# onucharles/tensorized-rnn

Measured on AMD Instinct MI355X. Metric: timesteps/sec/GPU (batch=64) TT-LSTM h=256 ncores=3 rank=8, higher is better.
Workload: dtype f32 (2xfp16 operands, fp32 accumulate)

## Files before the change

### tensorized-rnn_amd/csrc/ttrnn_f10_dev.h

```cpp
#pragma once
#include <hip/hip_runtime.h>
#include "ttrnn_core.h"
#include "ttrnn_mfma.h"
#include "ttrnn_split.h"
#include "ttrnn_f10.h"

namespace ttrnn {

template <class S, int KS>
constexpr size_t f10_lds_bytes() {
  return 2 * sizeof(float) * F10<S>::H + 2 * 3 * 2 * (size_t)F10<S>::H + 2 * 3 * (size_t)F10<S>::PLANE +
         (KS == 2 ? F10<S>::MT * 64 * sizeof(f32x4) : 0);
}

template <class S>
__device__ __forceinline__ void f10_load_w2(xbf8& a1, xbf8& a2, const float* packed, int mt, int lane) {
  using F = F10<S>;
  const int r = lane & 15, q = lane >> 4;
  const float* W2 = packed + woff_of<S>(2);
#pragma unroll
  for (int e = 0; e < 8; ++e) {
    __bf16 p0, p1, p2;
    split3(e < F::J2 ? W2[e * F::M2 + 16 * mt + r] : 0.f, p0, p1, p2);
    a1[e] = (q & 1) ? p1 : p0;
// ... 221 lines not shown
#pragma unroll
  for (int e = 0; e < 4; ++e) d[e] = ln.live ? d[e] : 0u;
  const xh8 bfrag = __builtin_bit_cast(xh8, u32x4{d[0], d[1], d[2], d[3]});
  f32x4 acc[NP];
#pragma unroll
  for (int p = 0; p < NP; ++p) acc[p] = __builtin_amdgcn_mfma_f32_16x16x32_f16(a1[p], bfrag, f32x4{0.f, 0.f, 0.f, 0.f}, 0, 0, 0);
#pragma unroll
  for (int p = 0; p < NP; ++p) acc[p] = __builtin_amdgcn_mfma_f32_16x16x32_f16(a2[p], bfrag, acc[p], 0, 0, 0);
#pragma unroll
  for (int p = 0; p < NP; ++p) store_split4_h(img, F::PLANE, ln.soff[p], acc[p]);
}
template <class S>
__device__ __forceinline__ void f10p_s2_lds(const xh8* afr, int lane, const F10pLane<S>& ln, unsigned pk, _Float16* img) {
  using F = F10<S>;
  constexpr int NP = F10P<S>::NP;
  unsigned d[4];
#pragma unroll
  for (int e = 0; e < 4; ++e) d[e] = (unsigned)__builtin_amdgcn_ds_bpermute(ln.gsrc + 4 * e, (int)pk);
#pragma unroll
  for (int e = 0; e < 4; ++e) d[e] = ln.live ? d[e] : 0u;
  const xh8 bfrag = __builtin_bit_cast(xh8, u32x4{d[0], d[1], d[2], d[3]});
  constexpr int GP = NP < 3 ? NP : 3;
  static_assert(NP % GP == 0, "pair groups");
#pragma unroll
  for (int p0 = 0; p0 < NP; p0 += GP) {
    xh8 fa[GP], fb[GP];
#pragma unroll
    for (int p = 0; p < GP; ++p) {
      fa[p] = afr[(2 * (p0 + p)) * 64 + lane];
      fb[p] = afr[(2 * (p0 + p) + 1) * 64 + lane];
    }
    f32x4 acc[GP];
#pragma unroll
    for (int p = 0; p < GP; ++p) acc[p] = __builtin_amdgcn_mfma_f32_16x16x32_f16(fa[p], bfrag, f32x4{0.f, 0.f, 0.f, 0.f}, 0, 0, 0);
#pragma unroll
    for (int p = 0; p < GP; ++p) acc[p] = __builtin_amdgcn_mfma_f32_16x16x32_f16(fb[p], bfrag, acc[p], 0, 0, 0);
#pragma unroll
    for (int p = 0; p < GP; ++p) store_split4_h(img, F::PLANE, ln.soff[p0 + p], acc[p]);
  }
}
__device__ __forceinline__ unsigned f10p_pack(float hscaled) {
  _Float16 p0, p1;
  split2h(hscaled, p0, p1);
  return (unsigned)__builtin_bit_cast(unsigned short, p0) | ((unsigned)__builtin_bit_cast(unsigned short, p1) << 16);
}

template <class S>
__global__ void __launch_bounds__(256) k_f10h_scale(const float* __restrict__ packed, int* __restrict__ hdr) {
  using F = F10<S>;
  static_assert(F::I2 <= 16 && F::R2 <= 16 && F::K % 64 == 0, "one workgroup (blockIdx.x) per row of the fused core: launch F::M of them");
  __shared__ unsigned mx[32];
  __shared__ int eu[16], ev[16];
  const int tid = threadIdx.x, lane = tid & 63, wave = tid >> 6;
  const float* W2 = packed + woff_of<S>(2);
  if (tid < 32) mx[tid] = 0u;
  __syncthreads();
  for (int i = tid; i < F::J2 * F::M2; i += 256)
    atomicMax(&mx[(i % F::M2) / F::R2], __float_as_uint(fabsf(W2[i])));
  __syncthreads();
  if (tid < 16) eu[tid] = tid < F::I2 ? -f10h_expo(__uint_as_float(mx[tid])) : 0;
  __syncthreads();
  for (int i = tid; i < F::J2 * F::M2; i += 256) {
    const int m2 = i % F::M2;
    atomicMax(&mx[16 + m2 % F::R2], __float_as_uint(fabsf(W2[i]) * ldexpf(1.f, eu[m2 / F::R2])));
  }
  __syncthreads();
  if (tid < 16) ev[tid] = tid < F::R2 ? -f10h_expo(__uint_as_float(mx[16 + tid])) : 0;
  __syncthreads();
  __shared__ float red[4];
  const int m = blockIdx.x;
  const int i0 = m / F::I1, i1 = m % F::I1;
  const float* W0 = packed + woff_of<S>(0);
  const float* W1 = packed + woff_of<S>(1);
  float best = 0.f;
  for (int k = tid; k < F::K; k += 256) {
    const int r2 = k % F::R2, row2 = k / F::R2;
    const int j1 = row2 % F::J1, j0 = row2 / F::J1;
    const float* w1p = W1 + (j1 * F::R2 + r2) * (F::I1 * F::R1) + i1 * F::R1;
    float v = 0.f;
    for (int r1 = 0; r1 < F::R1; ++r1) v = fmaf(W0[(j0 * F::R1 + r1) * F::I0 + i0], w1p[r1], v);
    best = fmaxf(best, fabsf(v) * ldexpf(1.f, -ev[r2]));
  }
#pragma unroll
  for (int o = 32; o > 0; o >>= 1) best = fmaxf(best, __shfl_xor(best, o));
  if (lane == 0) red[wave] = best;
  __syncthreads();
  if (tid == 0) hdr[F10H_EP + m] = 12 - f10h_expo(fmaxf(fmaxf(red[0], red[1]), fmaxf(red[2], red[3])));
  if (blockIdx.x == 0 && tid < 16) {
    hdr[F10H_EU + tid] = eu[tid];
    hdr[F10H_EV + tid] = ev[tid];
  }
}

static constexpr int F10T_ROW_EXP = 10;
static constexpr int F10T_ACC_EXP = 16;
static constexpr float F10T_HSC = 16.0f;
template <class S>
__device__ __forceinline__ int f10t_build_w10(xh8 (&w10)[8][2], const float* packed, const float* __restrict__ hdr, int wave, int lane) {
  using F = F10<S>;
  static_assert(F::R2 == 8 && F::J0 == 4 && F::J1 == 8 && F::R1 == 8 && F::M == 64 && F::MPG == 16, "H = 256, r = 8");
  const int c = lane & 15, q = lane >> 4;
  const int* ev = reinterpret_cast<const int*>(hdr) + F10H_EV;
  const int g = c & 3, m = F::MPG * g + 4 * wave + (c >> 2);
  const int i0 = m / F::I1, i1 = m % F::I1;
  const float* W0 = packed + woff_of<S>(0);
  const float* W1 = packed + woff_of<S>(1);
  float w0[F::R1];
#pragma unroll
  for (int r1 = 0; r1 < F::R1; ++r1) w0[r1] = W0[(q * F::R1 + r1) * F::I0 + i0];
  auto entry = [&](int e, int r2) {
    const float* w1p = W1 + (e * F::R2 + r2) * (F::I1 * F::R1) + i1 * F::R1;
    float v = 0.f;
#pragma unroll
    for (int r1 = 0; r1 < F::R1; ++r1) v = fmaf(w0[r1], w1p[r1], v);
    return v;
  };
  float best = 0.f;
#pragma unroll
  for (int r2 = 0; r2 < F::R2; ++r2) {
    float l1 = 0.f;
#pragma unroll
    for (int e = 0; e < 8; ++e) l1 += fabsf(entry(e, r2));
    l1 += __shfl_xor(l1, 16);
    l1 += __shfl_xor(l1, 32);
    best = fmaxf(best, l1 * ldexpf(1.f, -ev[r2]));
  }
  const int ept = F10T_ROW_EXP - f10h_expo(best);
  const float gf = g == 2 ? 2.8853900817779268f : -1.4426950408889634f;
#pragma unroll
  for (int r2 = 0; r2 < F::R2; ++r2) {
    const float sc = gf * ldexpf(1.f, ept - ev[r2]);
#pragma unroll
    for (int e = 0; e < 8; ++e) {
      _Float16 p0, p1;
      split2h_scaled(entry(e, r2), sc, p0, p1);
      w10[r2][0][e] = p0; w10[r2][1][e] = p1;
    }
  }
  return ept;
}
__device__ __forceinline__ F10hScales f10t_scales(const float* __restrict__ hdr, int ept_mine, int lane) {
  const int* e = reinterpret_cast<const int*>(hdr);
  const int c = lane & 15, q = lane >> 4;
  const int eu = e[F10H_EU + c];
  F10hScales r;
#pragma unroll
  for (int j = 0; j < 4; ++j) {
    const int s = __shfl(ept_mine, 4 * q + j) + eu + F10T_ACC_EXP;
    r.pre[j] = ldexpf(1.f, s);
    r.un[j] = ldexpf(1.f, -s);
  }
  return r;
}
template <class S>
__device__ __forceinline__ void f10t_load_g2(xh8 (&g2)[2][2], const float* packed, int lane, const float* __restrict__ hdr) {
  using F = F10<S>;
  const int c = lane & 15, q = lane >> 4;
  const float* W2 = packed + woff_of<S>(2);
  const int* e = reinterpret_cast<const int*>(hdr);
#pragma unroll
  for (int kb = 0; kb < 2; ++kb)
#pragma unroll
    for (int j = 0; j < 8; ++j) {
      const int r2 = 2 * kb + (j >> 2) + 4 * (q >> 1), j2 = 4 * (q & 1) + (j & 3);
      _Float16 p0, p1;
      split2h(W2[j2 * F::M2 + c * F::R2 + r2] * ldexpf(1.f, 12 + e[F10H_EU + c] + e[F10H_EV + r2]), p0, p1);
      g2[kb][0][j] = p0; g2[kb][1][j] = p1;
    }
}

}
```

### tensorized-rnn_amd/csrc/ttrnn_fast_f10t.hip

```cpp
#include <hip/hip_runtime.h>
#include <stdlib.h>
#include "ttrnn_core.h"
#include "ttrnn_launch.h"
#include "ttrnn_opts.h"
#include "ttrnn_mfma.h"
#include "ttrnn_split.h"
#include "ttrnn_f10.h"
#include "ttrnn_f10_dev.h"

namespace ttrnn {

static constexpr size_t F10T_LDS_BYTES = 2 * 2 * 8 * 32 * sizeof(_Float16) + 64;

template <class S, bool H0, bool OUT, bool IN1, bool DIAG = false>
__global__ void __launch_bounds__(256, 2) k_lstm_fwd_f10t(int B, int T, GinSrc gs, const float* __restrict__ h0,
                                                          const float* __restrict__ c0, const float* __restrict__ packed_hid,
                                                          const float* __restrict__ hdr,
                                                          const float* __restrict__ bias_hid, float* __restrict__ out,
                                                          float* __restrict__ hT, float* __restrict__ cT,
                                                          float* __restrict__ reserve) {
  static_assert(f10_ok<S>(), "shape not supported by the fused-core kernel");
  using F = F10<S>;
  static_assert(F::MT == 4 && F::ROWS2 == 32 && F::J2 == 8 && F::R2 == 8 && F::I2 == 16 && F::M == 64, "H = 256, r = 8");
  constexpr int H = F::H;
  constexpr int PAR = 2 * 8 * 32;

  extern __shared__ __attribute__((aligned(16))) unsigned char smem_t[];
  _Float16* himg = reinterpret_cast<_Float16*>(smem_t);
  float* scratch = reinterpret_cast<float*>(himg + 2 * PAR);

  const int tid = threadIdx.x, lane = tid & 63;
  const int wave = __builtin_amdgcn_readfirstlane(tid >> 6);
  xh8 w10[F::R2][2];
  const F10hScales fsc = f10t_scales(hdr, f10t_build_w10<S>(w10, packed_hid, hdr, wave, lane), lane);
  const float hsc = F10T_HSC;
  const f32x4 psc = fsc.pre, usc = fsc.un;
  const int c = lane & 15, q = lane >> 4;
  const size_t b = blockIdx.x;

  xh8 g2[2][2];
  f10t_load_g2<S>(g2, packed_hid, lane, hdr);

  const float* __restrict__ gin = gs.gin;
  const float* __restrict__ xs = reinterpret_cast<const float*>(gs.x);
  constexpr bool in1 = IN1;
  const int hd = (4 * wave + q) * F::I2 + c;
  const int hoff = (hd & 7) * 32 + (hd >> 3);
  float hst = H0 ? h0[b * H + hd] : 0.f;
  float cst = c0 ? c0[b * H + hd] : 0.f;
  float h0sc = 1.0f, h0un = 1.0f;
  if constexpr (H0) {
    const int e0 = f10h_h0_expo<4>(hst, scratch, wave, lane);
    h0sc = ldexpf(1.f, -e0); h0un = ldexpf(1.f, e0);
  }
  f32x4 bh = f32x4{0.f, 0.f, 0.f, 0.f}, gi = bh, vv = bh, bb = bh;
  const f32x4 gsc = f32x4{-1.4426950408889634f, 2.8853900817779268f, -1.4426950408889634f, -1.4426950408889634f} *
                    f32x4{psc[0], psc[2], psc[1], psc[3]};
  XChunk<float> xq;
  xq.cur = 0.f; xq.nxt = 0.f;
  if (in1) xq.init(xs, b * T, T, lane);
  if (bias_hid) bh = f32x4{bias_hid[hd], bias_hid[2 * H + hd], bias_hid[H + hd], bias_hid[3 * H + hd]};
  if (T > 0) {
    if (in1) {
      bb = *reinterpret_cast<const f32x4*>(gin + (H + hd) * 4);
      vv = (*reinterpret_cast<const f32x4*>(gin + hd * 4) - bb) * gsc;
      bb = (bb + bh) * gsc;
    } else {
      gi = *reinterpret_cast<const f32x4*>(gin + ((b * T) * H + hd) * 4);
    }
  }
  {
    _Float16 p0, p1;
    split2h(hst * (hsc * h0sc), p0, p1);
    himg[hoff] = p0; himg[256 + hoff] = p1;
  }
  __builtin_amdgcn_s_waitcnt(0x0F70);
  lds_barrier();

  unsigned long long seg[8] = {0, 0, 0, 0, 0, 0, 0, 0};
  unsigned long long last_ = 0;
  if constexpr (DIAG) last_ = stamp();
  f32x4 us_t = usc * h0un;
  float ps_t = h0sc;
  for (int t = 0; t < T; ++t) {
    const _Float16* hp = himg + (t & 1) * PAR;
    _Float16* hn = himg + ((t + 1) & 1) * PAR;
    const xh8 ha = *reinterpret_cast<const xh8*>(hp + c * 32 + 8 * q);
    f32x4 d[F::R2];
#pragma unroll
    for (int r = 0; r < F::R2; ++r) d[r] = __builtin_amdgcn_mfma_f32_16x16x32_f16(ha, w10[r][0], f32x4{0.f, 0.f, 0.f, 0.f}, 0, 0, 0);
#pragma unroll
    for (int r = 0; r < F::R2; ++r) d[r] = __builtin_amdgcn_mfma_f32_16x16x32_f16(ha, w10[r][1], d[r], 0, 0, 0);
    if constexpr (DIAG) {
#pragma unroll
      for (int r = 0; r < F::R2; ++r) asm volatile("" : "+v"(d[r]));
    }
    TT_STAMP(0)
    unsigned a0[2][4], a1[2][4];
#pragma unroll
    for (int p = 0; p < 4; ++p) {
      f32x4 s;
#pragma unroll
      for (int j = 0; j < 4; ++j) {
        const auto r = __builtin_amdgcn_permlane32_swap(__float_as_uint(d[p][j]), __float_as_uint(d[p + 4][j]), false, false);
        s[j] = __uint_as_float(r[0]) + __uint_as_float(r[1]);
      }
      split_pair_h(s[0], s[1], a0[p >> 1][2 * (p & 1)], a1[p >> 1][2 * (p & 1)]);
      split_pair_h(s[2], s[3], a0[p >> 1][2 * (p & 1) + 1], a1[p >> 1][2 * (p & 1) + 1]);
    }
    if constexpr (DIAG) {
#pragma unroll
      for (int kb = 0; kb < 2; ++kb)
#pragma unroll
        for (int j = 0; j < 4; ++j) asm volatile("" : "+v"(a0[kb][j]), "+v"(a1[kb][j]));
    }
    TT_STAMP(1)
    const size_t bt = b * T + t;
    f32x4 acc;
    {
      f32x4 pre = in1 ? bb + xq.at(t) * vv : (gi + bh) * gsc;
      if constexpr (H0) pre = pre * ps_t;
      f32x4 acc_lo = f32x4{0.f, 0.f, 0.f, 0.f}, acc_hi = f32x4{pre[0], pre[2], pre[1], pre[3]};
#pragma unroll
      for (int kb = 0; kb < 2; ++kb) {
        const xh8 d0 = __builtin_bit_cast(xh8, u32x4{a0[kb][0], a0[kb][1], a0[kb][2], a0[kb][3]});
        const xh8 d1 = __builtin_bit_cast(xh8, u32x4{a1[kb][0], a1[kb][1], a1[kb][2], a1[kb][3]});
        acc_lo = __builtin_amdgcn_mfma_f32_16x16x32_f16(d0, g2[kb][1], acc_lo, 0, 0, 0);
        acc_lo = __builtin_amdgcn_mfma_f32_16x16x32_f16(d1, g2[kb][0], acc_lo, 0, 0, 0);
        acc_hi = __builtin_amdgcn_mfma_f32_16x16x32_f16(d0, g2[kb][0], acc_hi, 0, 0, 0);
      }
      const f32x4 un = H0 ? us_t : usc;
      acc = acc_hi * un + acc_lo * un;
      if constexpr (DIAG) asm volatile("" : "+v"(acc));
    }
    TT_STAMP(2)
    const float ig = __builtin_amdgcn_rcpf(1.0f + __builtin_amdgcn_exp2f(acc[0]));
    const float fg = __builtin_amdgcn_rcpf(1.0f + __builtin_amdgcn_exp2f(acc[1]));
    const float gg = 1.0f - 2.0f * __builtin_amdgcn_rcpf(1.0f + __builtin_amdgcn_exp2f(acc[2]));
    const float og = __builtin_amdgcn_rcpf(1.0f + __builtin_amdgcn_exp2f(acc[3]));
    const float cy = fg * cst + ig * gg;
    const float hy = og * ftanh(cy);
    cst = cy;
    hst = hy;
    {
      _Float16 p0, p1;
      split2h(hy * hsc, p0, p1);
      hn[hoff] = p0; hn[256 + hoff] = p1;
    }
    if constexpr (OUT) out[bt * H + hd] = hy;
    if (reserve) {
      *reinterpret_cast<f32x4*>(reserve + res_gate(bt, H, hd)) = f32x4{ig, gg, fg, og};
      reserve[res_cell((size_t)B * T, bt, H, hd)] = cy;
    }
    if (!in1 && t + 1 < T) gi = *reinterpret_cast<const f32x4*>(gin + ((bt + 1) * H + hd) * 4);
    if (in1) xq.advance(xs, b * T, T, t, lane);
    us_t = usc; ps_t = 1.0f;
    TT_STAMP(3)
    lds_barrier();
    TT_STAMP(4)
  }
  if (hT) hT[b * H + hd] = hst;
  if (cT) cT[b * H + hd] = cst;
  if constexpr (DIAG) {
    if (lane == 0 && reserve && b < 8) {
      unsigned long long* dst = reinterpret_cast<unsigned long long*>(reserve) + (b * 8 + wave) * 8;
#pragma unroll
      for (int i = 0; i < 8; ++i) dst[i] = seg[i];
    }
  }
}

bool f10t_available(const RnnShape& rs) {
  if (opt(OPT_DEV2) & 2048) return false;
  return shape_matches<ShpH256R8L>(rs.hid_s) && rs.B <= device_cu_count();
}

int launch_rnn_fwd_f10_t(const RnnShape& rs, GinSrc gin, const void* h0, const void* c0, const float* packed_hid,
                         const void* ws, const float* bias_hid, void* out, void* hT, void* cT, float* reserve,
                         hipStream_t stream) {
  using S = ShpH256R8L;
  if (!shape_matches<S>(rs.hid_s)) return TTRNN_ERR_UNSUPPORTED;
  const float* hdr = reinterpret_cast<const float*>(ws);
  auto kern = gin.in1 ? (out ? (h0 ? k_lstm_fwd_f10t<S, true, true, true> : k_lstm_fwd_f10t<S, false, true, true>)
                             : (h0 ? k_lstm_fwd_f10t<S, true, false, true> : k_lstm_fwd_f10t<S, false, false, true>))
                      : (out ? (h0 ? k_lstm_fwd_f10t<S, true, true, false> : k_lstm_fwd_f10t<S, false, true, false>)
                             : (h0 ? k_lstm_fwd_f10t<S, true, false, false> : k_lstm_fwd_f10t<S, false, false, false>));
  if (opt(OPT_DIAG) && reserve && out && !h0)
    kern = gin.in1 ? k_lstm_fwd_f10t<S, false, true, true, true> : k_lstm_fwd_f10t<S, false, true, false, true>;
  hipLaunchKernelGGL(kern, dim3(rs.B), dim3(256), F10T_LDS_BYTES, stream, rs.B, rs.T, gin, (const float*)h0,
                     (const float*)c0, packed_hid, hdr, bias_hid, (float*)out, (float*)hT, (float*)cT, reserve);
  return hipGetLastError() == hipSuccess ? TTRNN_OK : TTRNN_ERR_LAUNCH;
}

}
```

### tensorized-rnn_amd/csrc/ttrnn_launch.h

```cpp
#pragma once
#include <hip/hip_runtime.h>
#include "ttrnn_core.h"

namespace ttrnn {

unsigned* device_status_ptr();


inline int device_cu_count() {
  static int cached[16] = {0};
  int dev = 0;
  if (hipGetDevice(&dev) != hipSuccess) {
    (void)hipGetLastError();
    return 256;
  }
  if (dev < 0 || dev >= 16) dev = 0;
  if (cached[dev] == 0) {
    int v = 256;
    if (hipDeviceGetAttribute(&v, hipDeviceAttributeMultiprocessorCount, dev) != hipSuccess) (void)hipGetLastError();
    cached[dev] = v > 0 ? v : 256;
  }
  return cached[dev];
}

int ensure_dynamic_lds(const void* fn, size_t bytes);
bool resident_at_once(const void* fn, int block_threads, size_t dyn_lds, long blocks);

struct GinSrc {
  const float* gin;
  const void* x;
  int in1;
  const int* run_if = nullptr;
  unsigned* status = nullptr;
};

struct LinPlan {
  int nb;
  int bs;
  int ss;
  int grid;
  bool w_lds;
  bool buf_global;
  bool buf_mixed;
  bool acc_lds;
  bool acc_slab;
  bool acc_fixed;
  size_t slab_off;
  size_t lds_bytes, ws_bytes;
};

struct RnnPlan {
  int nb, grid;
  bool w_lds, buf_global;
  size_t lds_bytes, ws_bytes;
};

LinPlan plan_ttlinear_fwd(const TtShape& s, int64_t n_rows);
LinPlan plan_ttlinear_bwd(const TtShape& s, int64_t n_rows, bool fixed_order = false);
RnnPlan plan_rnn_generic(const RnnShape& rs, bool backward);

const void* unit_rows_ptr(int dtype);
size_t in1_reduce_part_bytes(int out);
int launch_in1_reduce(int dtype, int dy_dtype, int64_t n_rows, int out, const void* x, const void* dy, float* dv,
                      float* db, float* part, hipStream_t stream);
int launch_pack(const TtShape& s, const void* const* cores, const int64_t* strides, int dtype, float* packed,
                hipStream_t stream);
int launch_pack2(const TtShape& sa, const void* const* cores_a, const int64_t* strides_a, float* packed_a,
                 const TtShape& sb, const void* const* cores_b, const int64_t* strides_b, float* packed_b, int dtype,
                 hipStream_t stream);
int launch_unpack(const TtShape& s, const float* packed_grad, void* const* grads, const int64_t* strides, int dtype,
                  hipStream_t stream);
int launch_ttlinear_fwd(const TtShape& s, const LinPlan& p, int dtype, int64_t n_rows, const float* packed,
                        const void* bias, const void* x, void* y, void* ws, hipStream_t stream, int ilv_h = 0,
                        int ilv_mode = 0, int epi = 0, float* aux = nullptr);
int launch_ttlinear_bwd(const TtShape& s, const LinPlan& p, int dtype, int dy_dtype, int64_t n_rows, const float* packed,
                        const void* x, const void* dy, void* dx, float* d_packed, float* d_bias, void* ws,
                        hipStream_t stream);
int launch_rnn_fwd_generic(const RnnShape& rs, const RnnPlan& p, int dtype, const void* x, const void* h0,
                           const void* c0, const float* packed_in, const void* bias_in, const float* packed_hid,
                           const void* bias_hid, void* out, void* hT, void* cT, float* reserve, void* ws,
                           hipStream_t stream, const int* lens = nullptr);
int launch_rnn_bwd_generic(const RnnShape& rs, const RnnPlan& p, int dtype, const void* out, const void* h0,
                           const void* c0, const float* packed_hid, const float* reserve, const void* d_out,
                           const void* d_hT, const void* d_cT, float* dg_in, float* dg_hid, void* d_h0, void* d_c0,
                           void* ws, hipStream_t stream, float* dstate = nullptr);

bool fast_rnn_fwd_available(const RnnShape& rs, int dtype);
int launch_rnn_fwd_fast(const RnnShape& rs, int dtype, GinSrc gin, const void* h0, const void* c0,
                        const float* packed_hid, const void* bias_hid, void* out, void* hT, void* cT, float* reserve,
                        hipStream_t stream);

bool fast_ttlinear_fwd_available(const TtShape& s, int dtype, int ilv_h);
int launch_ttlinear_fwd_fast(const TtShape& s, int dtype, bool y_f32, int64_t n_rows, const float* packed,
                             const void* bias, const void* x, void* y, int ilv_h, int ilv_mode, hipStream_t stream);

bool fast_rnn_fwd_bf16_available(const RnnShape& rs, int dtype);
int launch_rnn_fwd_bf16(const RnnShape& rs, GinSrc gin, const void* h0, const void* c0,
                        const float* packed_hid, const void* bias_hid, void* out, void* hT, void* cT, float* reserve,
                        hipStream_t stream);

bool f10_rnn_fwd_available(const RnnShape& rs, int dtype);
size_t f10_workspace_bytes(const RnnShape& rs, int dtype);
int launch_rnn_fwd_f10(const RnnShape& rs, GinSrc gin, const void* h0, const void* c0, const float* packed_hid,
                       const void* bias_hid, void* out, void* hT, void* cT, float* reserve, void* ws,
                       hipStream_t stream, int phase = 0);

bool f2_rnn_fwd_available(const RnnShape& rs, int dtype);
size_t f2_workspace_bytes(const RnnShape& rs, int dtype);
int launch_rnn_fwd_f2(const RnnShape& rs, GinSrc gin, const void* h0, const void* c0, const float* packed_hid,
                      const void* bias_hid, void* out, void* hT, void* cT, float* reserve, void* ws, hipStream_t stream, int phase);
bool f2_rnn_bwd_available(const RnnShape& rs, int dtype);
size_t f2_rnn_bwd_workspace_bytes(const RnnShape& rs, int dtype);
int launch_rnn_bwd_f2(const RnnShape& rs, const void* c0, const float* packed_hid, const float* reserve, const void* d_out,
                      const void* d_hT, const void* d_cT, float* dg_in, float* dg_hid, void* d_h0, void* d_c0, void* ws,
                      hipStream_t stream);

size_t f10gq_workspace_bytes();
bool f10gq_available(const RnnShape& rs, int dtype);
int launch_gru_fwd_f10gq(const RnnShape& rs, GinSrc gin, const void* h0, const float* packed_hid, const void* bias_hid,
                         void* out, void* hT, float* reserve, void* ws, hipStream_t stream, int phase);
bool f10_setup_available(const RnnShape& rs, int dtype);
int launch_f10_setup(const RnnShape& rs, const void* const* cores_in, const int64_t* strides_in, const void* bias_in,
                     const void* const* cores_hid, const int64_t* strides_hid, float* packed_in, float* packed_hid, float* gin,
                     void* ws, hipStream_t stream);
bool f10s_available(const RnnShape& rs, bool with_h0);
int launch_rnn_fwd_f10_s(const RnnShape& rs, GinSrc gin, const void* h0, const void* c0, const float* packed_hid, const void* ws,
                         const float* bias_hid, void* out, void* hT, void* cT, float* reserve, hipStream_t stream);
size_t f10gh_workspace_bytes(const RnnShape& rs);
bool f10gh_available(const RnnShape& rs, int dtype);
int launch_gru_fwd_f10gh(const RnnShape& rs, GinSrc gin, const void* h0, const float* packed_hid, const void* bias_hid, void* out,
                         void* hT, float* reserve, void* ws, hipStream_t stream, int phase);
bool f10n_available(const RnnShape& rs, int dtype);
size_t f10n_workspace_bytes(const RnnShape& rs);
int launch_lstm_fwd_f10n(const RnnShape& rs, GinSrc gin, const float* bilv, const void* h0, const void* c0, const float* packed_hid,
                         void* out, void* hT, void* cT, float* reserve, void* ws, hipStream_t stream);
bool f10g5_available(const RnnShape& rs, int dtype);
size_t f10g5_workspace_bytes(const RnnShape& rs);
int launch_gru_fwd_f10g5(const RnnShape& rs, const float* gin, const void* h0, const float* packed_hid, void* out, void* hT,
                         float* reserve, void* ws, hipStream_t stream);
int launch_gru_fwd_f10gh_g2(const RnnShape& rs, GinSrc src, const float* bilv, const void* h0, const float* packed_hid, void* out,
                            void* hT, float* reserve, void* ws, hipStream_t stream);
bool f10gh_own_plan(const RnnShape& rs);
int launch_rnn_fwd_f10_nb2(const RnnShape& rs, GinSrc gin, const void* h0, const void* c0, const float* packed_hid,
                           const void* wfrag, const float* bias_hid, void* out, void* hT, void* cT, float* reserve,
                           hipStream_t stream);
bool f10t_available(const RnnShape& rs);
bool f10_fwd_takes_f10t(const RnnShape& rs);
int launch_rnn_fwd_f10_t(const RnnShape& rs, GinSrc gin, const void* h0, const void* c0, const float* packed_hid,
                         const void* ws, const float* bias_hid, void* out, void* hT, void* cT, float* reserve,
                         hipStream_t stream);
int launch_rnn_fwd_f10_q(const RnnShape& rs, GinSrc gin, const void* h0, const void* c0, const float* packed_hid,
                           const void* wfrag, const float* bias_hid, void* out, void* hT, void* cT, float* reserve,
                           hipStream_t stream);

bool f10_h512_fwd_available(const RnnShape& rs, int dtype);
size_t f10_h512_workspace_bytes();
int launch_rnn_fwd_f10_h512(const RnnShape& rs, const float* gin, const void* h0, const void* c0, const float* packed_hid,
                            void* out, void* hT, void* cT, float* reserve, void* ws, hipStream_t stream);

bool f10x_rnn_fwd_available(const RnnShape& rs, int dtype);
int launch_rnn_fwd_f10x(const RnnShape& rs, GinSrc gin, const void* h0, const void* c0, const float* packed_hid,
                        const void* bias_hid, void* out, void* hT, void* cT, float* reserve, void* ws,
                        hipStream_t stream);

bool f10_ttlinear_fwd_available(const TtShape& s, int dtype, int ilv_h, int ilv_mode);
size_t f10_ttlinear_workspace_bytes(const TtShape& s, int dtype, int ilv_h, int ilv_mode);
int launch_ttlinear_fwd_f10(const TtShape& s, int64_t n_rows, const float* packed, const void* bias, const void* x,
                            void* y, void* ws, hipStream_t stream);

bool gemm_split_ok(int K, int M);
size_t gemm_split_identity_bytes(int K);
size_t gemm_split_dense_bytes(int K, int M);
size_t gemm_split_plane_bytes(int K, int M);
int launch_fill_identity(int dtype, int K, void* id, hipStream_t stream);
int launch_gemm_split_prep(const float* WG, int K, int M, void* planes, hipStream_t stream, bool transposed = false);
int launch_gemm_split(int dtype, int64_t n_rows, int K, int M, const void* x, const void* planes, const void* bias,
                      int Hb, float* y, hipStream_t stream, const float* bias_ilv = nullptr);

size_t gemm_half_scratch_bytes(int64_t n_rows, int K, int M);
bool gemm3_ok(int64_t n_rows, int K, int M);
size_t gemm3_xplane_bytes(int64_t n_rows, int K);
int launch_gemm3h(int dtype, int64_t n_rows, int K, int M, const void* x, const void* planes, void* scratch, void* xplanes,
                  const void* bias, int Hb, float* y, hipStream_t stream, const float* bias_ilv);
bool gemm_use_half(int64_t n_rows, int K, int M);
int launch_gemm_half_prep(const float* WG, int K, int M, void* planes, void* scratch, hipStream_t stream,
                          bool transposed = false);
int launch_gemm_half(int dtype, int64_t n_rows, int K, int M, const void* x, const void* planes, void* scratch,
                     const void* bias, int Hb, float* y, hipStream_t stream, const float* bias_ilv = nullptr,
                     const float* rowmax = nullptr);

bool dense_wgrad_ok(int in, int out);
bool dense_wgrad_shift_ok(int64_t n_rows, int64_t shift_T);
int launch_dense_wgrad(int dtype, int64_t n_rows, int in, int out, const void* x, const float* dy, float* dW,
                       float* d_bias, hipStream_t stream, bool split, float* scratch, const unsigned* x_colmax = nullptr,
                       const unsigned* dy_colmax = nullptr, int shift_T = 0, const void* shift_first = nullptr);
size_t dense_wgrad_scratch_bytes(int in, int out);

bool big_rnn_fwd_available(const RnnShape& rs, int dtype);
size_t big_rnn_fwd_workspace(const RnnShape& rs);
int launch_rnn_fwd_big(const RnnShape& rs, int dtype, const void* x, const void* h0, const void* c0,
                       const float* packed_in, const void* bias_in, const float* packed_hid, const void* bias_hid,
                       void* out, void* hT, void* cT, float* reserve, void* workspace, hipStream_t stream);

size_t bigh_workspace_bytes();
bool bigh_pair_resident(int dtype, int B);
int launch_lstm_fwd_big2h(const RnnShape& rs, int dtype, const float* gin, const void* h0, const void* c0,
                          const float* m2_hid, const void* bias_in, const void* bias_hid, void* out, void* hT, void* cT,
                          float* reserve, unsigned long long* hxb, void* scratch, hipStream_t stream);

size_t bigbh_workspace_bytes();
bool bigbh_pair_resident(int dtype, int B);
const float* bigbh_guard_rows(const void* scratch, int* n_rows);
int launch_lstm_bwd_big2h(const RnnShape& rs, int dtype, const void* c0, const float* fragT, const float* reserve,
                          const void* d_out, const void* d_hT, const void* d_cT, float* dg_in, void* d_h0, void* d_c0,
                          unsigned long long* hxb, void* scratch, hipStream_t stream, unsigned* colmax = nullptr);

bool big_rnn_bwd_available(const RnnShape& rs, int dtype);
size_t big_rnn_bwd_workspace(const RnnShape& rs);
int launch_rnn_bwd_big(const RnnShape& rs, int dtype, const void* c0, const float* packed_hid, const float* reserve,
                       const void* d_out, const void* d_hT, const void* d_cT, float* dg_in, float* dg_hid, void* d_h0,
                       void* d_c0, void* ws, hipStream_t stream, float* stats = nullptr);
bool big_ttlinear_bwd_available(const TtShape& s, int dtype, int dy_dtype);
size_t big_ttlinear_bwd_workspace_bytes(const TtShape& s);
int launch_ttlinear_bwd_big(const TtShape& s, int dtype, int64_t n_rows, const float* packed, const void* x,
                            const void* dy, void* dx, float* d_packed, float* d_bias, void* ws, hipStream_t stream,
                            const unsigned* x_colmax = nullptr, const unsigned* dy_colmax = nullptr, int shift_T = 0,
                            const void* shift_first = nullptr);

bool g2_rnn_available(const RnnShape& rs, int dtype);
bool g2_rnn_fwd_paired(const RnnShape& rs);
bool g2_rnn_bwd_available(const RnnShape& rs, int dtype);
size_t g2_rnn_fwd_workspace(const RnnShape& rs);
size_t g2_rnn_bwd_workspace(const RnnShape& rs);
int launch_rnn_fwd_g2(const RnnShape& rs, int dtype, const void* x, const void* h0, const void* c0, const float* packed_in,
                      const void* bias_in, const float* packed_hid, const void* bias_hid, void* out, void* hT, void* cT,
                      float* reserve, void* workspace, hipStream_t stream, const int* lens = nullptr);
bool g2_rnn_varlen_available(const RnnShape& rs, int dtype);
size_t g2_rnn_fwd_varlen_workspace(const RnnShape& rs);
int launch_rnn_bwd_g2(const RnnShape& rs, int dtype, const void* out, const void* h0, const void* c0, const float* packed_hid,
                      const float* reserve, const void* d_out, const void* d_hT, const void* d_cT, float* dg_in,
                      float* dg_hid, void* d_h0, void* d_c0, void* ws, hipStream_t stream, float* dstate = nullptr,
                      float* stats = nullptr);
bool g2_rnn_bwd_colmax(const RnnShape& rs);

bool fast_rnn_bwd_available(const RnnShape& rs, int dtype);
int launch_rnn_bwd_fast(const RnnShape& rs, int dtype, const void* out, const void* h0, const void* c0,
                        const float* packed_hid, const float* reserve, const void* d_out, const void* d_hT,
                        const void* d_cT, float* dg_in, float* dg_hid, void* d_h0, void* d_c0, hipStream_t stream);

bool f10_rnn_bwd_available(const RnnShape& rs, int dtype);
size_t f10_rnn_bwd_workspace_bytes(const RnnShape& rs, int dtype);
struct BwdStats {
  const void* x = nullptr;
  float* part = nullptr;
  unsigned* colmax = nullptr;
  float* rowmax = nullptr;
};
int launch_bwd_stats_finish(int cell, int Bn, int GH, const float* part, float* stats, hipStream_t stream);
size_t bwd_stats_part_bytes(const RnnShape& rs);
int launch_rnn_bwd_f10(const RnnShape& rs, int dtype, const void* out, const void* h0, const void* c0,
                       const float* packed_hid, const float* reserve, const void* d_out, const void* d_hT,
                       const void* d_cT, float* dg_in, float* dg_hid, void* d_h0, void* d_c0, void* ws,
                       hipStream_t stream, const void* x_in1 = nullptr, float* stats = nullptr);

bool f10bh_available(const RnnShape& rs, int dtype);
bool f10bh_h512_available(const RnnShape& rs, int dtype);
size_t f10n_unjoined_floats(int cell);
int launch_f10n_unjoin(const RnnShape& rs, const float* packed_hid, float* pg, hipStream_t stream);
bool f10n_shape_matches(const RnnShape& rs);
bool f10n_bwd_available(const RnnShape& rs, int dtype);
size_t f10n_bwd_workspace_bytes(const RnnShape& rs);
int launch_rnn_bwd_f10n(const RnnShape& rs, const void* out, const void* h0, const void* c0, const float* packed_hid,
                        const float* reserve, const void* d_out, const void* d_hT, const void* d_cT, float* dg_in, float* dg_hid,
                        void* d_h0, void* d_c0, void* ws, hipStream_t stream, float* stats);
size_t f10bh_h512_workspace_bytes();
int launch_rnn_bwd_f10_h512(const RnnShape& rs, const void* out, const void* h0, const void* c0, const float* packed_hid,
                            const float* reserve, const void* d_out, const void* d_hT, const void* d_cT, float* dg_in, float* dg_hid,
                            void* d_h0, void* d_c0, void* ws, hipStream_t stream, float* stats);
size_t proj3_workspace_bytes(const TtShape& s);
int launch_proj3(const TtShape& s, const float* packed, const float* dW, float* d_packed, void* ws, hipStream_t stream);
size_t f10bh_workspace_bytes(const RnnShape& rs);
int launch_lstm_bwd_f10h(const RnnShape& rs, const void* c0, const float* packed_hid, const float* reserve,
                         const void* d_out, const void* d_hT, const void* d_cT, float* dg_in, float* dg_hid, void* d_h0,
                         void* d_c0, void* ws, unsigned long long* diag, hipStream_t stream, const BwdStats& bs);

int launch_gru_bwd_f10h(const RnnShape& rs, int dtype, const void* out, const void* h0, const float* packed_hid,
                        const float* reserve, const void* d_out, const void* d_hT, float* dg_in, float* dg_hid, void* d_h0,
                        void* ws, hipStream_t stream, const BwdStats& bs);

size_t f10b_fragment_bytes(const TtShape& s);
int launch_f10b_prep(const TtShape& s, const float* packed, void* wfrag, hipStream_t stream, float* zero = nullptr,
                     int zero_n = 0);

bool f10_ttlinear_wgrad_available(const TtShape& s, int dtype, int dy_dtype);
size_t f10_ttlinear_wgrad_workspace_bytes(const TtShape& s);
bool f10_ttlinear_wgrad_has_dx(const TtShape& s);
int launch_ttlinear_wgrad_f10(const TtShape& s, int dtype, int64_t n_rows, const float* packed, const void* x,
                              const void* dy, void* dx, float* d_packed, float* d_bias, void* ws, hipStream_t stream);

bool fast_ttlinear_bwd_available(const TtShape& s, int dtype, int dy_dtype);
int launch_ttlinear_bwd_fast(const TtShape& s, int dtype, int dy_dtype, int64_t n_rows, const float* packed,
                             const void* x, const void* dy, void* dx, float* d_packed, float* d_bias,
                             hipStream_t stream);
// ... 24 lines not shown
```

Baseline: 2.033 million.

## Re-layout the h image so core-1 MFMA outputs feed core-2 without lane swaps

Adds an ADJ variant of the fused TT-LSTM kernel that stores the split fp16 hidden state in a padded, XOR-swizzled LDS layout (48-element rows). The rows are ordered so the partial sums of each first-stage MFMA tile can be reduced inside the lane, dropping the permlane32_swap reduction, and the core-2 weight fragments are reindexed to match. The next step's h fragment is also read right after the barrier, at the end of the loop, instead of at the top of the next iteration. This removes cross-lane shuffles and LDS bank conflicts from the serial per-timestep critical path. The old layout stays reachable behind an option bit, and the change is a new default that would be wrong if the reordered indices do not match.

After: 2.419 million (median of 6 runs). 19.0% higher.

```diff
diff --git a/tensorized-rnn_amd/csrc/ttrnn_f10_dev.h b/tensorized-rnn_amd/csrc/ttrnn_f10_dev.h
--- a/tensorized-rnn_amd/csrc/ttrnn_f10_dev.h
+++ b/tensorized-rnn_amd/csrc/ttrnn_f10_dev.h
@@ -397,7 +397,11 @@
   }
   return r;
 }
-template <class S>
+static constexpr int F10T_ROW = 48;
+__device__ __forceinline__ constexpr int f10t_img_off(int row, int k) {
+  return row * F10T_ROW + 8 * ((k >> 3) ^ ((row >> 2) & 3)) + (k & 7);
+}
+template <class S, bool ADJ = false>
 __device__ __forceinline__ void f10t_load_g2(xh8 (&g2)[2][2], const float* packed, int lane, const float* __restrict__ hdr) {
   using F = F10<S>;
   const int c = lane & 15, q = lane >> 4;
@@ -407,7 +411,7 @@
   for (int kb = 0; kb < 2; ++kb)
 #pragma unroll
     for (int j = 0; j < 8; ++j) {
-      const int r2 = 2 * kb + (j >> 2) + 4 * (q >> 1), j2 = 4 * (q & 1) + (j & 3);
+      const int r2 = ADJ ? 4 * kb + (j >> 1) : 2 * kb + (j >> 2) + 4 * (q >> 1), j2 = ADJ ? 2 * q + (j & 1) : 4 * (q & 1) + (j & 3);
       _Float16 p0, p1;
       split2h(W2[j2 * F::M2 + c * F::R2 + r2] * ldexpf(1.f, 12 + e[F10H_EU + c] + e[F10H_EV + r2]), p0, p1);
       g2[kb][0][j] = p0; g2[kb][1][j] = p1;
diff --git a/tensorized-rnn_amd/csrc/ttrnn_f10t_kernel.h b/tensorized-rnn_amd/csrc/ttrnn_f10t_kernel.h
--- /dev/null
+++ b/tensorized-rnn_amd/csrc/ttrnn_f10t_kernel.h
@@ -0,0 +1,203 @@
+#pragma once
+#include <hip/hip_runtime.h>
+#include <stdlib.h>
+#include "ttrnn_core.h"
+#include "ttrnn_launch.h"
+#include "ttrnn_opts.h"
+#include "ttrnn_mfma.h"
+#include "ttrnn_split.h"
+#include "ttrnn_f10.h"
+#include "ttrnn_f10_dev.h"
+
+namespace ttrnn {
+
+template <bool ADJ>
+static constexpr size_t F10T_LDS_BYTES = 2 * (ADJ ? 16 * F10T_ROW : 2 * 8 * 32) * sizeof(_Float16) + 64;
+
+template <class S, bool H0, bool OUT, bool IN1, bool ADJ, bool DIAG = false>
+__global__ void __launch_bounds__(256, 2) k_lstm_fwd_f10t(int B, int T, GinSrc gs, const float* __restrict__ h0,
+                                                          const float* __restrict__ c0, const float* __restrict__ packed_hid,
+                                                          const float* __restrict__ hdr,
+                                                          const float* __restrict__ bias_hid, float* __restrict__ out,
+                                                          float* __restrict__ hT, float* __restrict__ cT,
+                                                          float* __restrict__ reserve) {
+  static_assert(f10_ok<S>(), "shape not supported by the fused-core kernel");
+  using F = F10<S>;
+  static_assert(F::MT == 4 && F::ROWS2 == 32 && F::J2 == 8 && F::R2 == 8 && F::I2 == 16 && F::M == 64, "H = 256, r = 8");
+  constexpr int H = F::H;
+  constexpr int PAR = ADJ ? 16 * F10T_ROW : 2 * 8 * 32;
+  constexpr int PIECE1 = ADJ ? F10T_ROW : 8 * 32;
+
+  extern __shared__ __attribute__((aligned(16))) unsigned char smem_t[];
+  _Float16* himg = reinterpret_cast<_Float16*>(smem_t);
+  float* scratch = reinterpret_cast<float*>(himg + 2 * PAR);
+
+  const int tid = threadIdx.x, lane = tid & 63;
+  const int wave = __builtin_amdgcn_readfirstlane(tid >> 6);
+  xh8 w10[F::R2][2];
+  const F10hScales fsc = f10t_scales(hdr, f10t_build_w10<S>(w10, packed_hid, hdr, wave, lane), lane);
+  const float hsc = F10T_HSC;
+  const f32x4 psc = fsc.pre, usc = fsc.un;
+  const int c = lane & 15, q = lane >> 4;
+  const size_t b = blockIdx.x;
+
+  xh8 g2[2][2];
+  f10t_load_g2<S, ADJ>(g2, packed_hid, lane, hdr);
+
+  const float* __restrict__ gin = gs.gin;
+  const float* __restrict__ xs = reinterpret_cast<const float*>(gs.x);
+  constexpr bool in1 = IN1;
+  const int hd = (4 * wave + q) * F::I2 + c;
+  const int hoff = ADJ ? f10t_img_off(2 * (hd & 7), hd >> 3) : (hd & 7) * 32 + (hd >> 3);
+  const int aoff = ADJ ? f10t_img_off(c, 8 * q) : c * 32 + 8 * q;
+  float hst = H0 ? h0[b * H + hd] : 0.f;
+  float cst = c0 ? c0[b * H + hd] : 0.f;
+  float h0sc = 1.0f, h0un = 1.0f;
+  if constexpr (H0) {
+    const int e0 = f10h_h0_expo<4>(hst, scratch, wave, lane);
+    h0sc = ldexpf(1.f, -e0); h0un = ldexpf(1.f, e0);
+  }
+  f32x4 bh = f32x4{0.f, 0.f, 0.f, 0.f}, gi = bh, vv = bh, bb = bh;
+  const f32x4 gsc = f32x4{-1.4426950408889634f, 2.8853900817779268f, -1.4426950408889634f, -1.4426950408889634f} *
+                    f32x4{psc[0], psc[2], psc[1], psc[3]};
+  XChunk<float> xq;
+  xq.cur = 0.f; xq.nxt = 0.f;
+  if (in1) xq.init(xs, b * T, T, lane);
+  if (bias_hid) bh = f32x4{bias_hid[hd], bias_hid[2 * H + hd], bias_hid[H + hd], bias_hid[3 * H + hd]};
+  if (T > 0) {
+    if (in1) {
+      bb = *reinterpret_cast<const f32x4*>(gin + (H + hd) * 4);
+      vv = (*reinterpret_cast<const f32x4*>(gin + hd * 4) - bb) * gsc;
+      bb = (bb + bh) * gsc;
+    } else {
+      gi = *reinterpret_cast<const f32x4*>(gin + ((b * T) * H + hd) * 4);
+    }
+  }
+  {
+    _Float16 p0, p1;
+    split2h(hst * (hsc * h0sc), p0, p1);
+    himg[hoff] = p0; himg[PIECE1 + hoff] = p1;
+  }
+  __builtin_amdgcn_s_waitcnt(0x0F70);
+  lds_barrier();
+
+  unsigned long long seg[8] = {0, 0, 0, 0, 0, 0, 0, 0};
+  unsigned long long last_ = 0;
+  if constexpr (DIAG) last_ = stamp();
+  f32x4 us_t = usc * h0un;
+  float ps_t = h0sc;
+  xh8 ha;
+  if constexpr (ADJ) ha = *reinterpret_cast<const xh8*>(himg + aoff);
+  for (int t = 0; t < T; ++t) {
+    const _Float16* hp = himg + (t & 1) * PAR;
+    _Float16* hn = himg + ((t + 1) & 1) * PAR;
+    if constexpr (!ADJ) ha = *reinterpret_cast<const xh8*>(hp + aoff);
+    f32x4 d[F::R2];
+#pragma unroll
+    for (int r = 0; r < F::R2; ++r) d[r] = __builtin_amdgcn_mfma_f32_16x16x32_f16(ha, w10[r][0], f32x4{0.f, 0.f, 0.f, 0.f}, 0, 0, 0);
+#pragma unroll
+    for (int r = 0; r < F::R2; ++r) d[r] = __builtin_amdgcn_mfma_f32_16x16x32_f16(ha, w10[r][1], d[r], 0, 0, 0);
+    if constexpr (DIAG) {
+#pragma unroll
+      for (int r = 0; r < F::R2; ++r) asm volatile("" : "+v"(d[r]));
+    }
+    TT_STAMP(0)
+    unsigned a0[2][4], a1[2][4];
+    if constexpr (ADJ) {
+#pragma unroll
+      for (int r = 0; r < F::R2; ++r)
+        split_pair_h(d[r][0] + d[r][1], d[r][2] + d[r][3], a0[r >> 2][r & 3], a1[r >> 2][r & 3]);
+    } else {
+#pragma unroll
+      for (int p = 0; p < 4; ++p) {
+        f32x4 s;
+#pragma unroll
+        for (int j = 0; j < 4; ++j) {
+          const auto r = __builtin_amdgcn_permlane32_swap(__float_as_uint(d[p][j]), __float_as_uint(d[p + 4][j]), false, false);
+          s[j] = __uint_as_float(r[0]) + __uint_as_float(r[1]);
+        }
+        split_pair_h(s[0], s[1], a0[p >> 1][2 * (p & 1)], a1[p >> 1][2 * (p & 1)]);
+        split_pair_h(s[2], s[3], a0[p >> 1][2 * (p & 1) + 1], a1[p >> 1][2 * (p & 1) + 1]);
+      }
+    }
+    if constexpr (DIAG) {
+#pragma unroll
+      for (int kb = 0; kb < 2; ++kb)
+#pragma unroll
+        for (int j = 0; j < 4; ++j) asm volatile("" : "+v"(a0[kb][j]), "+v"(a1[kb][j]));
+    }
+    TT_STAMP(1)
+    const size_t bt = b * T + t;
+    f32x4 acc;
+    {
+      f32x4 pre = in1 ? bb + xq.at(t) * vv : (gi + bh) * gsc;
+      if constexpr (H0) pre = pre * ps_t;
+      f32x4 acc_lo = f32x4{0.f, 0.f, 0.f, 0.f}, acc_hi = f32x4{pre[0], pre[2], pre[1], pre[3]};
+#pragma unroll
+      for (int kb = 0; kb < 2; ++kb) {
+        const xh8 d0 = __builtin_bit_cast(xh8, u32x4{a0[kb][0], a0[kb][1], a0[kb][2], a0[kb][3]});
+        const xh8 d1 = __builtin_bit_cast(xh8, u32x4{a1[kb][0], a1[kb][1], a1[kb][2], a1[kb][3]});
+        acc_lo = __builtin_amdgcn_mfma_f32_16x16x32_f16(d0, g2[kb][1], acc_lo, 0, 0, 0);
+        acc_lo = __builtin_amdgcn_mfma_f32_16x16x32_f16(d1, g2[kb][0], acc_lo, 0, 0, 0);
+        acc_hi = __builtin_amdgcn_mfma_f32_16x16x32_f16(d0, g2[kb][0], acc_hi, 0, 0, 0);
+      }
+      const f32x4 un = H0 ? us_t : usc;
+      acc = acc_hi * un + acc_lo * un;
+      if constexpr (DIAG) asm volatile("" : "+v"(acc));
+    }
+    TT_STAMP(2)
+    const float ig = __builtin_amdgcn_rcpf(1.0f + __builtin_amdgcn_exp2f(acc[0]));
+    const float fg = __builtin_amdgcn_rcpf(1.0f + __builtin_amdgcn_exp2f(acc[1]));
+    const float gg = 1.0f - 2.0f * __builtin_amdgcn_rcpf(1.0f + __builtin_amdgcn_exp2f(acc[2]));
+    const float og = __builtin_amdgcn_rcpf(1.0f + __builtin_amdgcn_exp2f(acc[3]));
+    const float cy = fg * cst + ig * gg;
+    const float hy = og * ftanh(cy);
+    cst = cy;
+    hst = hy;
+    {
+      _Float16 p0, p1;
+      split2h(hy * hsc, p0, p1);
+      hn[hoff] = p0; hn[PIECE1 + hoff] = p1;
+    }
+    if constexpr (OUT) out[bt * H + hd] = hy;
+    if (reserve) {
+      *reinterpret_cast<f32x4*>(reserve + res_gate(bt, H, hd)) = f32x4{ig, gg, fg, og};
+      reserve[res_cell((size_t)B * T, bt, H, hd)] = cy;
+    }
+    if (!in1 && t + 1 < T) gi = *reinterpret_cast<const f32x4*>(gin + ((bt + 1) * H + hd) * 4);
+    if (in1) xq.advance(xs, b * T, T, t, lane);
+    us_t = usc; ps_t = 1.0f;
+    TT_STAMP(3)
+    lds_barrier();
+    if constexpr (ADJ) {
+      ha = *reinterpret_cast<const xh8*>(hn + aoff);
+      __builtin_amdgcn_sched_barrier(0);
+    }
+    TT_STAMP(4)
+  }
+  if (hT) hT[b * H + hd] = hst;
+  if (cT) cT[b * H + hd] = cst;
+  if constexpr (DIAG) {
+    if (lane == 0 && reserve && b < 8) {
+      unsigned long long* dst = reinterpret_cast<unsigned long long*>(reserve) + (b * 8 + wave) * 8;
+#pragma unroll
+      for (int i = 0; i < 8; ++i) dst[i] = seg[i];
+    }
+  }
+}
+
+template <class S, bool ADJ>
+static int launch_f10t(const RnnShape& rs, GinSrc gin, const void* h0, const void* c0, const float* packed_hid, const float* hdr,
+                       const float* bias_hid, void* out, void* hT, void* cT, float* reserve, hipStream_t stream) {
+  auto kern = gin.in1 ? (out ? (h0 ? k_lstm_fwd_f10t<S, true, true, true, ADJ> : k_lstm_fwd_f10t<S, false, true, true, ADJ>)
+                             : (h0 ? k_lstm_fwd_f10t<S, true, false, true, ADJ> : k_lstm_fwd_f10t<S, false, false, true, ADJ>))
+                      : (out ? (h0 ? k_lstm_fwd_f10t<S, true, true, false, ADJ> : k_lstm_fwd_f10t<S, false, true, false, ADJ>)
+                             : (h0 ? k_lstm_fwd_f10t<S, true, false, false, ADJ> : k_lstm_fwd_f10t<S, false, false, false, ADJ>));
+  if (opt(OPT_DIAG) && reserve && out && !h0)
+    kern = gin.in1 ? k_lstm_fwd_f10t<S, false, true, true, ADJ, true> : k_lstm_fwd_f10t<S, false, true, false, ADJ, true>;
+  hipLaunchKernelGGL(kern, dim3(rs.B), dim3(256), F10T_LDS_BYTES<ADJ>, stream, rs.B, rs.T, gin, (const float*)h0,
+                     (const float*)c0, packed_hid, hdr, bias_hid, (float*)out, (float*)hT, (float*)cT, reserve);
+  return hipGetLastError() == hipSuccess ? TTRNN_OK : TTRNN_ERR_LAUNCH;
+}
+
+}
diff --git a/tensorized-rnn_amd/csrc/ttrnn_fast_f10t.hip b/tensorized-rnn_amd/csrc/ttrnn_fast_f10t.hip
--- a/tensorized-rnn_amd/csrc/ttrnn_fast_f10t.hip
+++ b/tensorized-rnn_amd/csrc/ttrnn_fast_f10t.hip
@@ -1,174 +1,6 @@
-#include <hip/hip_runtime.h>
-#include <stdlib.h>
-#include "ttrnn_core.h"
-#include "ttrnn_launch.h"
-#include "ttrnn_opts.h"
-#include "ttrnn_mfma.h"
-#include "ttrnn_split.h"
-#include "ttrnn_f10.h"
-#include "ttrnn_f10_dev.h"
+#include "ttrnn_f10t_kernel.h"
 
 namespace ttrnn {
-
-static constexpr size_t F10T_LDS_BYTES = 2 * 2 * 8 * 32 * sizeof(_Float16) + 64;
-
-template <class S, bool H0, bool OUT, bool IN1, bool DIAG = false>
-__global__ void __launch_bounds__(256, 2) k_lstm_fwd_f10t(int B, int T, GinSrc gs, const float* __restrict__ h0,
-                                                          const float* __restrict__ c0, const float* __restrict__ packed_hid,
-                                                          const float* __restrict__ hdr,
-                                                          const float* __restrict__ bias_hid, float* __restrict__ out,
-                                                          float* __restrict__ hT, float* __restrict__ cT,
-                                                          float* __restrict__ reserve) {
-  static_assert(f10_ok<S>(), "shape not supported by the fused-core kernel");
-  using F = F10<S>;
-  static_assert(F::MT == 4 && F::ROWS2 == 32 && F::J2 == 8 && F::R2 == 8 && F::I2 == 16 && F::M == 64, "H = 256, r = 8");
-  constexpr int H = F::H;
-  constexpr int PAR = 2 * 8 * 32;
-
-  extern __shared__ __attribute__((aligned(16))) unsigned char smem_t[];
-  _Float16* himg = reinterpret_cast<_Float16*>(smem_t);
-  float* scratch = reinterpret_cast<float*>(himg + 2 * PAR);
-
-  const int tid = threadIdx.x, lane = tid & 63;
-  const int wave = __builtin_amdgcn_readfirstlane(tid >> 6);
-  xh8 w10[F::R2][2];
-  const F10hScales fsc = f10t_scales(hdr, f10t_build_w10<S>(w10, packed_hid, hdr, wave, lane), lane);
-  const float hsc = F10T_HSC;
-  const f32x4 psc = fsc.pre, usc = fsc.un;
-  const int c = lane & 15, q = lane >> 4;
-  const size_t b = blockIdx.x;
-
-  xh8 g2[2][2];
-  f10t_load_g2<S>(g2, packed_hid, lane, hdr);
-
-  const float* __restrict__ gin = gs.gin;
-  const float* __restrict__ xs = reinterpret_cast<const float*>(gs.x);
-  constexpr bool in1 = IN1;
-  const int hd = (4 * wave + q) * F::I2 + c;
-  const int hoff = (hd & 7) * 32 + (hd >> 3);
-  float hst = H0 ? h0[b * H + hd] : 0.f;
-  float cst = c0 ? c0[b * H + hd] : 0.f;
-  float h0sc = 1.0f, h0un = 1.0f;
-  if constexpr (H0) {
-    const int e0 = f10h_h0_expo<4>(hst, scratch, wave, lane);
-    h0sc = ldexpf(1.f, -e0); h0un = ldexpf(1.f, e0);
-  }
-  f32x4 bh = f32x4{0.f, 0.f, 0.f, 0.f}, gi = bh, vv = bh, bb = bh;
-  const f32x4 gsc = f32x4{-1.4426950408889634f, 2.8853900817779268f, -1.4426950408889634f, -1.4426950408889634f} *
-                    f32x4{psc[0], psc[2], psc[1], psc[3]};
-  XChunk<float> xq;
-  xq.cur = 0.f; xq.nxt = 0.f;
-  if (in1) xq.init(xs, b * T, T, lane);
-  if (bias_hid) bh = f32x4{bias_hid[hd], bias_hid[2 * H + hd], bias_hid[H + hd], bias_hid[3 * H + hd]};
-  if (T > 0) {
-    if (in1) {
-      bb = *reinterpret_cast<const f32x4*>(gin + (H + hd) * 4);
-      vv = (*reinterpret_cast<const f32x4*>(gin + hd * 4) - bb) * gsc;
-      bb = (bb + bh) * gsc;
-    } else {
-      gi = *reinterpret_cast<const f32x4*>(gin + ((b * T) * H + hd) * 4);
-    }
-  }
-  {
-    _Float16 p0, p1;
-    split2h(hst * (hsc * h0sc), p0, p1);
-    himg[hoff] = p0; himg[256 + hoff] = p1;
-  }
-  __builtin_amdgcn_s_waitcnt(0x0F70);
-  lds_barrier();
-
-  unsigned long long seg[8] = {0, 0, 0, 0, 0, 0, 0, 0};
-  unsigned long long last_ = 0;
-  if constexpr (DIAG) last_ = stamp();
-  f32x4 us_t = usc * h0un;
-  float ps_t = h0sc;
-  for (int t = 0; t < T; ++t) {
-    const _Float16* hp = himg + (t & 1) * PAR;
-    _Float16* hn = himg + ((t + 1) & 1) * PAR;
-    const xh8 ha = *reinterpret_cast<const xh8*>(hp + c * 32 + 8 * q);
-    f32x4 d[F::R2];
-#pragma unroll
-    for (int r = 0; r < F::R2; ++r) d[r] = __builtin_amdgcn_mfma_f32_16x16x32_f16(ha, w10[r][0], f32x4{0.f, 0.f, 0.f, 0.f}, 0, 0, 0);
-#pragma unroll
-    for (int r = 0; r < F::R2; ++r) d[r] = __builtin_amdgcn_mfma_f32_16x16x32_f16(ha, w10[r][1], d[r], 0, 0, 0);
-    if constexpr (DIAG) {
-#pragma unroll
-      for (int r = 0; r < F::R2; ++r) asm volatile("" : "+v"(d[r]));
-    }
-    TT_STAMP(0)
-    unsigned a0[2][4], a1[2][4];
-#pragma unroll
-    for (int p = 0; p < 4; ++p) {
-      f32x4 s;
-#pragma unroll
-      for (int j = 0; j < 4; ++j) {
-        const auto r = __builtin_amdgcn_permlane32_swap(__float_as_uint(d[p][j]), __float_as_uint(d[p + 4][j]), false, false);
-        s[j] = __uint_as_float(r[0]) + __uint_as_float(r[1]);
-      }
-      split_pair_h(s[0], s[1], a0[p >> 1][2 * (p & 1)], a1[p >> 1][2 * (p & 1)]);
-      split_pair_h(s[2], s[3], a0[p >> 1][2 * (p & 1) + 1], a1[p >> 1][2 * (p & 1) + 1]);
-    }
-    if constexpr (DIAG) {
-#pragma unroll
-      for (int kb = 0; kb < 2; ++kb)
-#pragma unroll
-        for (int j = 0; j < 4; ++j) asm volatile("" : "+v"(a0[kb][j]), "+v"(a1[kb][j]));
-    }
-    TT_STAMP(1)
-    const size_t bt = b * T + t;
-    f32x4 acc;
-    {
-      f32x4 pre = in1 ? bb + xq.at(t) * vv : (gi + bh) * gsc;
-      if constexpr (H0) pre = pre * ps_t;
-      f32x4 acc_lo = f32x4{0.f, 0.f, 0.f, 0.f}, acc_hi = f32x4{pre[0], pre[2], pre[1], pre[3]};
-#pragma unroll
-      for (int kb = 0; kb < 2; ++kb) {
-        const xh8 d0 = __builtin_bit_cast(xh8, u32x4{a0[kb][0], a0[kb][1], a0[kb][2], a0[kb][3]});
-        const xh8 d1 = __builtin_bit_cast(xh8, u32x4{a1[kb][0], a1[kb][1], a1[kb][2], a1[kb][3]});
-        acc_lo = __builtin_amdgcn_mfma_f32_16x16x32_f16(d0, g2[kb][1], acc_lo, 0, 0, 0);
-        acc_lo = __builtin_amdgcn_mfma_f32_16x16x32_f16(d1, g2[kb][0], acc_lo, 0, 0, 0);
-        acc_hi = __builtin_amdgcn_mfma_f32_16x16x32_f16(d0, g2[kb][0], acc_hi, 0, 0, 0);
-      }
-      const f32x4 un = H0 ? us_t : usc;
-      acc = acc_hi * un + acc_lo * un;
-      if constexpr (DIAG) asm volatile("" : "+v"(acc));
-    }
-    TT_STAMP(2)
-    const float ig = __builtin_amdgcn_rcpf(1.0f + __builtin_amdgcn_exp2f(acc[0]));
-    const float fg = __builtin_amdgcn_rcpf(1.0f + __builtin_amdgcn_exp2f(acc[1]));
-    const float gg = 1.0f - 2.0f * __builtin_amdgcn_rcpf(1.0f + __builtin_amdgcn_exp2f(acc[2]));
-    const float og = __builtin_amdgcn_rcpf(1.0f + __builtin_amdgcn_exp2f(acc[3]));
-    const float cy = fg * cst + ig * gg;
-    const float hy = og * ftanh(cy);
-    cst = cy;
-    hst = hy;
-    {
-      _Float16 p0, p1;
-      split2h(hy * hsc, p0, p1);
-      hn[hoff] = p0; hn[256 + hoff] = p1;
-    }
-    if constexpr (OUT) out[bt * H + hd] = hy;
-    if (reserve) {
-      *reinterpret_cast<f32x4*>(reserve + res_gate(bt, H, hd)) = f32x4{ig, gg, fg, og};
-      reserve[res_cell((size_t)B * T, bt, H, hd)] = cy;
-    }
-    if (!in1 && t + 1 < T) gi = *reinterpret_cast<const f32x4*>(gin + ((bt + 1) * H + hd) * 4);
-    if (in1) xq.advance(xs, b * T, T, t, lane);
-    us_t = usc; ps_t = 1.0f;
-    TT_STAMP(3)
-    lds_barrier();
-    TT_STAMP(4)
-  }
-  if (hT) hT[b * H + hd] = hst;
-  if (cT) cT[b * H + hd] = cst;
-  if constexpr (DIAG) {
-    if (lane == 0 && reserve && b < 8) {
-      unsigned long long* dst = reinterpret_cast<unsigned long long*>(reserve) + (b * 8 + wave) * 8;
-#pragma unroll
-      for (int i = 0; i < 8; ++i) dst[i] = seg[i];
-    }
-  }
-}
 
 bool f10t_available(const RnnShape& rs) {
   if (opt(OPT_DEV2) & 2048) return false;
@@ -180,16 +12,8 @@
                          hipStream_t stream) {
   using S = ShpH256R8L;
   if (!shape_matches<S>(rs.hid_s)) return TTRNN_ERR_UNSUPPORTED;
-  const float* hdr = reinterpret_cast<const float*>(ws);
-  auto kern = gin.in1 ? (out ? (h0 ? k_lstm_fwd_f10t<S, true, true, true> : k_lstm_fwd_f10t<S, false, true, true>)
-                             : (h0 ? k_lstm_fwd_f10t<S, true, false, true> : k_lstm_fwd_f10t<S, false, false, true>))
-                      : (out ? (h0 ? k_lstm_fwd_f10t<S, true, true, false> : k_lstm_fwd_f10t<S, false, true, false>)
-                             : (h0 ? k_lstm_fwd_f10t<S, true, false, false> : k_lstm_fwd_f10t<S, false, false, false>));
-  if (opt(OPT_DIAG) && reserve && out && !h0)
-    kern = gin.in1 ? k_lstm_fwd_f10t<S, false, true, true, true> : k_lstm_fwd_f10t<S, false, true, false, true>;
-  hipLaunchKernelGGL(kern, dim3(rs.B), dim3(256), F10T_LDS_BYTES, stream, rs.B, rs.T, gin, (const float*)h0,
-                     (const float*)c0, packed_hid, hdr, bias_hid, (float*)out, (float*)hT, (float*)cT, reserve);
-  return hipGetLastError() == hipSuccess ? TTRNN_OK : TTRNN_ERR_LAUNCH;
+  if (opt(OPT_DEV2) & 4096) return launch_rnn_fwd_f10_t_r7(rs, gin, h0, c0, packed_hid, ws, bias_hid, out, hT, cT, reserve, stream);
+  return launch_f10t<S, true>(rs, gin, h0, c0, packed_hid, reinterpret_cast<const float*>(ws), bias_hid, out, hT, cT, reserve, stream);
 }
 
 }
diff --git a/tensorized-rnn_amd/csrc/ttrnn_fast_f10t_r7.hip b/tensorized-rnn_amd/csrc/ttrnn_fast_f10t_r7.hip
--- /dev/null
+++ b/tensorized-rnn_amd/csrc/ttrnn_fast_f10t_r7.hip
@@ -0,0 +1,13 @@
+#include "ttrnn_f10t_kernel.h"
+
+namespace ttrnn {
+
+int launch_rnn_fwd_f10_t_r7(const RnnShape& rs, GinSrc gin, const void* h0, const void* c0, const float* packed_hid,
+                            const void* ws, const float* bias_hid, void* out, void* hT, void* cT, float* reserve,
+                            hipStream_t stream) {
+  using S = ShpH256R8L;
+  if (!shape_matches<S>(rs.hid_s)) return TTRNN_ERR_UNSUPPORTED;
+  return launch_f10t<S, false>(rs, gin, h0, c0, packed_hid, reinterpret_cast<const float*>(ws), bias_hid, out, hT, cT, reserve, stream);
+}
+
+}
diff --git a/tensorized-rnn_amd/csrc/ttrnn_launch.h b/tensorized-rnn_amd/csrc/ttrnn_launch.h
--- a/tensorized-rnn_amd/csrc/ttrnn_launch.h
+++ b/tensorized-rnn_amd/csrc/ttrnn_launch.h
@@ -149,6 +149,9 @@
 int launch_rnn_fwd_f10_t(const RnnShape& rs, GinSrc gin, const void* h0, const void* c0, const float* packed_hid,
                          const void* ws, const float* bias_hid, void* out, void* hT, void* cT, float* reserve,
                          hipStream_t stream);
+int launch_rnn_fwd_f10_t_r7(const RnnShape& rs, GinSrc gin, const void* h0, const void* c0, const float* packed_hid,
+                            const void* ws, const float* bias_hid, void* out, void* hT, void* cT, float* reserve,
+                            hipStream_t stream);
 int launch_rnn_fwd_f10_q(const RnnShape& rs, GinSrc gin, const void* h0, const void* c0, const float* packed_hid,
                            const void* wfrag, const float* bias_hid, void* out, void* hT, void* cT, float* reserve,
                            hipStream_t stream);
```
